# kfkq/DQMC

Measured on AMD Instinct MI355X. Metric: MC sweeps/sec, 2D Hubbard N=256 Ltau=200, higher is better.
Workload: dtype f64; 1 GPU; cfg3: 16x16 Hubbard U=8.0 beta=8.0 Ltau=200 n_stab=10 t=1 mu=-0.1; chains_per_gpu=1, n_chains_total=1, parallelism=independent chains, 1 gpu x 1 chain

## Files before the change

### dqmc_amd/abi.py

```python
from __future__ import annotations

import ctypes as C
import os
from typing import Optional, Tuple

import numpy as np

c_double_p = C.POINTER(C.c_double)
c_int64_p = C.POINTER(C.c_int64)
c_int32_p = C.POINTER(C.c_int32)
c_uint8_p = C.POINTER(C.c_uint8)
c_uint32_p = C.POINTER(C.c_uint32)
c_uint64_p = C.POINTER(C.c_uint64)


class Stats(C.Structure):
    _fields_ = [("acc_rate", C.c_double), ("max_err", C.c_double), ("sum_err", C.c_double),
                ("n_err", C.c_double), ("n_accepted", C.c_int64), ("n_proposed", C.c_int64)]

    @property
    def mean_err(self) -> float:
        return self.sum_err / self.n_err if self.n_err else 0.0


class DqmcError(RuntimeError):
    def __init__(self, code: int, msg: str):
        super().__init__(f"[{code}] {msg}")
        self.code = code


ABI_SYMBOLS = [
    "last_error", "backend", "device_count",
    "to_ldr", "ldr_mul_mat", "mat_mul_ldr", "ldr_mul_ldr", "inv_I_plus_ldr", "inv_I_plus_ldr_mul_ldr",
    "gemm", "rank1_update",
    "create", "create_batch", "n_chains", "destroy", "set_fields", "get_fields", "init", "get_G", "set_G", "get_logdet",
    "n_stack", "get_stack", "sweep_0_to_beta", "sweep_beta_to_0", "sync", "get_stats",
    "wrap_forward", "wrap_backward", "local_update_slice", "calculate_Bbar", "global_action", "set_checkerboard",
    "update_kernel_time", "set_profiling", "slice_path", "debug_snapshot", "bbar_rider_launches", "debug_gt_check",
    "measure_equal_time", "measure_accumulate", "measure_fetch",
    "sweep_unequal_time", "get_G_tau", "half_warp", "measure_unequal_time", "measure_unequal_fetch",
    "comm_unique_id", "comm_create_rccl", "comm_create_callbacks", "comm_destroy", "comm_rank", "comm_world_size",
    "comm_transport", "comm_barrier", "comm_allreduce_sum", "comm_selftest", "partner_rank", "replica_exchange_round",
    "replica_exchange_batch",
    "rng_seed", "rng_state", "rng_draw", "rng_fill_time",
]

UNIQUE_ID_BYTES = 128
SENDRECV_FN = C.CFUNCTYPE(C.c_int, C.c_void_p, C.c_void_p, C.c_void_p, C.c_size_t, C.c_int, C.c_int)


class ExchangeResult(C.Structure):
    _fields_ = [("partner", C.c_int), ("decider", C.c_int), ("accepted", C.c_int), ("pad", C.c_int),
                ("S", C.c_double), ("S_prime", C.c_double), ("S_partner", C.c_double), ("S_prime_partner", C.c_double),
# ... 69 lines not shown
            g("comm_create_callbacks").argtypes = [C.POINTER(C.c_void_p), C.c_int, C.c_int, SENDRECV_FN, C.c_void_p]
            g("comm_destroy").argtypes = [C.c_void_p]; g("comm_destroy").restype = None
            g("comm_rank").argtypes = [C.c_void_p]; g("comm_world_size").argtypes = [C.c_void_p]
            g("comm_transport").argtypes = [C.c_void_p]; g("comm_transport").restype = C.c_char_p
            g("comm_barrier").argtypes = [C.c_void_p]; g("comm_selftest").argtypes = [C.c_void_p]
            g("comm_allreduce_sum").argtypes = [C.c_void_p, c_double_p, C.c_int]
            g("partner_rank").argtypes = [C.c_int, C.c_int, C.c_int]
            g("replica_exchange_round").argtypes = [C.c_void_p, C.c_void_p, C.c_int, C.c_double, C.POINTER(ExchangeResult)]
        if self.has_symbol("replica_exchange_batch"):
            g("replica_exchange_batch").argtypes = [C.c_void_p, C.c_void_p, C.c_int, c_double_p, C.POINTER(ExchangeResult)]
        if self.has_symbol("rng_seed"):
            g("rng_seed").argtypes = [C.c_void_p, C.c_uint64, C.c_uint32, C.c_uint32]
            g("rng_state").argtypes = [C.c_void_p, c_uint64_p, c_uint32_p, c_uint32_p, C.POINTER(C.c_int)]
            g("rng_draw").argtypes = [C.c_void_p, C.c_uint32, c_int32_p, c_uint8_p, c_double_p]
            g("rng_fill_time").argtypes = [C.c_void_p, C.c_int, c_double_p]
        g("to_ldr").argtypes = [C.c_int] + [c_double_p] * 4
        g("ldr_mul_mat").argtypes = [C.c_int] + [c_double_p] * 7
        g("mat_mul_ldr").argtypes = [C.c_int] + [c_double_p] * 7
        g("ldr_mul_ldr").argtypes = [C.c_int] + [c_double_p] * 9
        g("inv_I_plus_ldr").argtypes = [C.c_int] + [c_double_p] * 5
        g("inv_I_plus_ldr_mul_ldr").argtypes = [C.c_int] + [c_double_p] * 7
        g("gemm").argtypes = [C.c_int, c_double_p, C.c_int, c_double_p, C.c_int, c_double_p]
        g("rank1_update").argtypes = [C.c_int, c_double_p, C.c_int, C.c_double]

    def _sym(self, name: str):
        return getattr(self._dll, self.prefix + name)

    def has_symbol(self, name: str) -> bool:
        return hasattr(self._dll, self.prefix + name)

# ... 41 lines not shown
        L1, d1, R1 = (_f64(x) for x in F1); L2, d2, R2 = (_f64(x) for x in F2); n = L1.shape[0]
        G = np.empty((n, n), order="F")
        self.check(self._sym("inv_I_plus_ldr_mul_ldr")(n, _p(L1), _p(d1), _p(R1), _p(L2), _p(d2), _p(R2), _p(G)))
        return G

    def gemm(self, A, B, transA: bool = False, transB: bool = False) -> np.ndarray:
        A = _f64(A); B = _f64(B); n = A.shape[0]
        Cm = np.empty((n, n), order="F")
        self.check(self._sym("gemm")(n, _p(A), int(transA), _p(B), int(transB), _p(Cm)))
        return Cm

    def rank1_update(self, G, i: int, delta: float) -> np.ndarray:
        G = np.array(G, dtype=np.float64, order="F", copy=True); n = G.shape[0]
        self.check(self._sym("rank1_update")(n, _p(G), int(i), float(delta)))
        return G

    def engine(self, *args, **kw) -> "Engine":
        return Engine(self, *args, **kw)

    def partner_rank(self, rank: int, world: int, attempt: int) -> int:
        return int(self._sym("partner_rank")(rank, world, attempt))

    def exchange_batch(self, engine: "Engine", attempt: int, u, comm: Optional["Comm"] = None) -> list:
        uv = np.ascontiguousarray(np.asarray(u, dtype=np.float64).reshape(-1))
        if uv.shape != (engine.C,):
            raise ValueError(f"u must have shape ({engine.C},), got {uv.shape}")
        res = (ExchangeResult * engine.C)()
        self.check(self._sym("replica_exchange_batch")(engine._h, comm._h if comm is not None else None, int(attempt), _p(uv), res))
        return list(res)

# ... 292 lines not shown
```

### dqmc_amd/csrc/common.h

```cpp
#pragma once

#include <hip/hip_runtime.h>
#include <cstdint>
#include <memory>
#include <string>

struct dqmc_engine;

namespace dq {

constexpr int WAVE = 64;

void set_error(const std::string& msg);
const char* get_error();

#define DQ_HIP(call)                                                                    \
    do {                                                                                \
        hipError_t _e = (call);                                                         \
        if (_e != hipSuccess) {                                                         \
            ::dq::set_error(std::string(#call) + ": " + hipGetErrorString(_e));         \
            return -2;                                              \
        }                                                                               \
    } while (0)

// ... 36 lines not shown

struct GemmDesc {
    CMat A, B;
    Mat C;
    Mat CT{nullptr, 0};
    CVec rs, ks, cs;
    int n = 0;
    int transA = 0;
    int accumulate = 0;
};
int launch_gemm(const GemmDesc& g, int n_chains, hipStream_t s);

int launch_build_expv(const int8_t* fields, long f_stride, int nt, int n, const double* tab_expv ,
                      double* expv, double* invexpv, long v_stride, int n_chains, hipStream_t s);
int launch_split_d(CVec d, Vec dl_inv, Vec ds, double* logsum, int n, int n_chains, hipStream_t s);
int launch_split_d2(CVec d1, Vec dl1, Vec ds1, CVec d2, Vec dl2, Vec ds2, int n, int n_chains, hipStream_t s);
int launch_measure_equal_time(CMat G, double* out, long out_stride, int L1, int L2, int accumulate, int n_chains, hipStream_t s);
int launch_measure_unequal_time(const double* Gtt, const double* Gt0, const double* G0t, double* out, long out_stride, int L1, int L2, int nt,
                                int accumulate, int n_chains, hipStream_t s);
int launch_axpb_identity(CMat in, Mat out, double a, double b, int n, int n_chains, hipStream_t s);
int launch_copy(CMat in, Mat out, long count, int n_chains, hipStream_t s);
int launch_set_identity(Mat out, int n, int n_chains, hipStream_t s);
int launch_transpose_scale(CMat in, Mat out, CVec rs, int n, int n_chains, hipStream_t s);
int launch_max_abs_diff(CMat A, CMat B, double* err, long err_stride, int n, int n_chains, hipStream_t s);
int launch_add_scaled_cols(CMat A, CMat B, CVec cs, Mat C, int n, int n_chains, hipStream_t s);
int launch_scale_rows(CMat in, CVec rs, Mat out, int n, int n_chains, hipStream_t s);
struct DevStats { double acc_rate, max_err, sum_err, n_err; long long n_accepted, n_proposed; };
int launch_fold_stats(DevStats* st, const int* acc, long acc_stride, int n_slices, const double* err, long err_stride, int n_err,
                      int n, int nt, int n_chains, hipStream_t s);

struct QrWork {
    double* tau; long tau_stride;
    int* jpvt; long jpvt_stride;
    unsigned long long* sync = nullptr; long sync_stride = 0;
    int* abort_words = nullptr;
    int* info = nullptr;
    double* pw = nullptr; long pw_stride = 0;
    bool pw_two_launch = false;
    int* pivpos = nullptr; long pivpos_stride = 0;
// ... 100 lines not shown
```

### dqmc_amd/csrc/elementwise.hip

```cpp
#include "common.h"
#include "wave.h"

namespace dq {

__global__ void build_expv_kernel(const int8_t* fields, long f_stride, long total, const double* tab,
                                  double* expv, double* invexpv, long v_stride) {
    const int c = blockIdx.y;
    const double* t = tab + (long)c * 8;
    for (long k = blockIdx.x * (long)blockDim.x + threadIdx.x; k < total; k += (long)gridDim.x * blockDim.x) {
        const int f = fields[(long)c * f_stride + k] & 3;
        expv[(long)c * v_stride + k] = t[f];
        invexpv[(long)c * v_stride + k] = t[4 + f];
    }
}
int launch_build_expv(const int8_t* fields, long f_stride, int nt, int n, const double* tab, double* expv, double* invexpv,
                      long v_stride, int n_chains, hipStream_t s) {
    const long total = (long)nt * n;
    dim3 grid((unsigned)((total + 255) / 256 > 512 ? 512 : (total + 255) / 256), n_chains);
    hipLaunchKernelGGL(build_expv_kernel, grid, dim3(256), 0, s, fields, f_stride, total, tab, expv, invexpv, v_stride);
    DQ_HIP(hipGetLastError());
    return 0;
}

__global__ void split_d_kernel(CVec d, Vec dl_inv, Vec ds, double* logsum, int n) {
// ... 3 lines not shown
    for (int i = threadIdx.x; i < n; i += blockDim.x) {
        const double v = dd[i];
        const bool large = v >= 1.0;
        dl_inv.at(c)[i] = large ? 1.0 / v : 1.0;
        ds.at(c)[i] = large ? 1.0 : v;
        if (large) ls += log(v);
    }
    if (logsum) {
        __shared__ double red[256];
        red[threadIdx.x] = ls;
        __syncthreads();
        for (int o = 128; o > 0; o >>= 1) { if ((int)threadIdx.x < o) red[threadIdx.x] += red[threadIdx.x + o]; __syncthreads(); }
        if (threadIdx.x == 0) logsum[c] = red[0];
    }
}
__global__ void split_d2_kernel(CVec d1, Vec dl1, Vec ds1, CVec d2, Vec dl2, Vec ds2, int n) {
    const int c = blockIdx.y;
    const double* dd = blockIdx.x ? d2.at(c) : d1.at(c);
    double* dl = blockIdx.x ? dl2.at(c) : dl1.at(c);
    double* ds = blockIdx.x ? ds2.at(c) : ds1.at(c);
    for (int i = threadIdx.x; i < n; i += blockDim.x) {
        const double v = dd[i];
        const bool large = v >= 1.0;
        dl[i] = large ? 1.0 / v : 1.0;
        ds[i] = large ? 1.0 : v;
    }
}
int launch_split_d2(CVec d1, Vec dl1, Vec ds1, CVec d2, Vec dl2, Vec ds2, int n, int n_chains, hipStream_t s) {
    hipLaunchKernelGGL(split_d2_kernel, dim3(2, n_chains), dim3(256), 0, s, d1, dl1, ds1, d2, dl2, ds2, n);
    DQ_HIP(hipGetLastError());
    return 0;
}
int launch_split_d(CVec d, Vec dl_inv, Vec ds, double* logsum, int n, int n_chains, hipStream_t s) {
    hipLaunchKernelGGL(split_d_kernel, dim3(1, n_chains), dim3(256), 0, s, d, dl_inv, ds, logsum, n);
    DQ_HIP(hipGetLastError());
    return 0;
}

__global__ void copy_kernel(CMat in, Mat out, long count) {
    const int c = blockIdx.y;
    const double* a = in.at(c); double* b = out.at(c);
    for (long k = blockIdx.x * (long)blockDim.x + threadIdx.x; k < count; k += (long)gridDim.x * blockDim.x) b[k] = a[k];
}
int launch_copy(CMat in, Mat out, long count, int n_chains, hipStream_t s) {
    long blocks = (count + 255) / 256; if (blocks > 1024) blocks = 1024;
    hipLaunchKernelGGL(copy_kernel, dim3((unsigned)blocks, n_chains), dim3(256), 0, s, in, out, count);
    DQ_HIP(hipGetLastError());
// ... 21 lines not shown
    const int tx = threadIdx.x & 31, ty = threadIdx.x >> 5;
    for (int r = ty; r < 32; r += 8) {
        const int i = ti * 32 + tx, j = tj * 32 + r;
        tile[r][tx] = (i < n && j < n) ? a[i + (long)n * j] : 0.0;
    }
    __syncthreads();
    for (int r = ty; r < 32; r += 8) {
        const int i = tj * 32 + tx, j = ti * 32 + r;
        if (i < n && j < n) {
            double v = tile[tx][r];
            if (rs.p) v *= rs.at(c)[i];
            o[i + (long)n * j] = v;
        }
    }
}
int launch_transpose_scale(CMat in, Mat out, CVec rs, int n, int n_chains, hipStream_t s) {
    const int tiles = (n + 31) / 32;
    hipLaunchKernelGGL(transpose_scale_kernel, dim3(tiles * tiles, n_chains), dim3(256), 0, s, in, out, rs, n, tiles);
    DQ_HIP(hipGetLastError());
    return 0;
}

__global__ __launch_bounds__(256) void max_abs_diff_kernel(CMat A, CMat B, double* err, long err_stride, int n) {
    const int c = blockIdx.y;
    const double* __restrict__ a = A.at(c); const double* __restrict__ b = B.at(c);
    const long total = (long)n * n;
    unsigned long long m = 0ULL;
    for (long k = (long)blockIdx.x * blockDim.x + threadIdx.x; k < total; k += (long)gridDim.x * blockDim.x) {
        const unsigned long long d = (unsigned long long)__double_as_longlong(fabs(a[k] - b[k]));
        m = d > m ? d : m;
// ... 1 lines not shown
    m = wave_max_u64(m);
    __shared__ unsigned long long red[4];
    if ((threadIdx.x & 63) == 0) red[threadIdx.x >> 6] = m;
    __syncthreads();
    if (threadIdx.x == 0) {
        unsigned long long r = red[0];
        for (int q = 1; q < 4; ++q) r = red[q] > r ? red[q] : r;
        atomicMax(reinterpret_cast<unsigned long long*>(err + (long)c * err_stride), r);
    }
}
int launch_max_abs_diff(CMat A, CMat B, double* err, long err_stride, int n, int n_chains, hipStream_t s) {
    const long total = (long)n * n;
    const long want = (total + 4095) / 4096;
    const int blocks = (int)(want < 1 ? 1 : (want > 16 ? 16 : want));
    hipLaunchKernelGGL(max_abs_diff_kernel, dim3(blocks, n_chains), dim3(256), 0, s, A, B, err, err_stride, n);
    DQ_HIP(hipGetLastError());
    return 0;
}

__global__ void add_scaled_cols_kernel(CMat A, CMat B, CVec cs, Mat C, int n) {
    const int c = blockIdx.y;
    const double* a = A.at(c); const double* b = B.at(c); double* o = C.at(c);
    const long total = (long)n * n;
    for (long k = blockIdx.x * (long)blockDim.x + threadIdx.x; k < total; k += (long)gridDim.x * blockDim.x) {
        double bv = b[k];
        if (cs.p) bv *= cs.at(c)[k / n];
        o[k] = a[k] + bv;
    }
}
int launch_add_scaled_cols(CMat A, CMat B, CVec cs, Mat C, int n, int n_chains, hipStream_t s) {
// ... 158 lines not shown
```

### dqmc_amd/csrc/engine.hip

```cpp
#include "common.h"
#include "../../include/dqmc_hip.h"

#include <cmath>
#include <cstdlib>
#include <cstring>
#include <map>
#include <memory>
#include <mutex>
#include <vector>

namespace dq {

static thread_local std::string g_err;
void set_error(const std::string& msg) { g_err = msg; }
const char* get_error() { return g_err.c_str(); }

int init_device_kernels(int device) {
    static std::mutex mu; static bool done[64] = {};
    std::lock_guard<std::mutex> lk(mu);
    if (device < 0 || device >= 64) { set_error("device ordinal out of range"); return -1; }
    if (done[device]) return 0;
    DQ_HIP(hipSetDevice(device));
    DQ_TRY(update_init_device()); DQ_TRY(update_sm_init_device()); DQ_TRY(qr_init_device()); DQ_TRY(qr_colown_init_device());
    done[device] = true;
// ... 189 lines not shown
        }
        DQ_TRY(launch_lu_blocked(M, lperm(), n, rowpos(), n, logdet_acc, 1, info(), n, C, stream));
        DQ_TRY(launch_lu_solve(M, lperm(), n, RHS, CVec(), 0, n, C, stream));
        *Y = RHS; return 0;
    }
    int inv_I_plus_ldr(LdrRef F, Mat G, double* logdet ) {
        DQ_TRY(launch_split_d(F.d, V(0), V(1), logdet, n, C, stream));
        Mat X; DQ_TRY(r_inverse_scaled(F, V(0), T(1), T(0), &X));
        DQ_TRY(launch_add_scaled_cols(X, F.L, V(1), T(2), n, C, stream));
        DQ_TRY(launch_transpose_scale(T(2), T(3), CVec(), n, C, stream));
        DQ_TRY(launch_transpose_scale(X, T(4), CVec(), n, C, stream));
        Mat Y; DQ_TRY(solve(T(3), T(4), T(0), logdet, &Y));
        return launch_transpose_scale(Y, G, CVec(), n, C, stream);
    }
    int inv_I_plus_ldr_mul_ldr(LdrRef F1, LdrRef F2, Mat G, Mat GT = Mat{nullptr, 0}) {
        DQ_TRY(launch_split_d2(F1.d, V(0), V(1), F2.d, V(2), V(3), n, C, stream));
        Mat X; DQ_TRY(r_inverse_scaled(F2, V(2), T(1), T(0), &X));
        DQ_TRY(gemm(F1.L, X, T(2), V(0), CVec(), CVec(), 1));
        DQ_TRY(gemm(F1.R, F2.L, T(2), V(1), CVec(), V(3), 0, 1));
        DQ_TRY(launch_transpose_scale(F1.L, T(3), V(0), n, C, stream));
        Mat Y; DQ_TRY(solve(T(2), T(3), T(0), nullptr, &Y));
        return gemm(X, Y, G, CVec(), CVec(), CVec(), 0, 0, GT);
    }
    int inv_invldr_plus_ldr(LdrRef F1, LdrRef F2, Mat G, bool negate) {
        DQ_TRY(launch_split_d(F1.d, V(0), V(1), nullptr, n, C, stream));
        DQ_TRY(launch_split_d(F2.d, V(2), V(3), nullptr, n, C, stream));
        Mat X; DQ_TRY(r_inverse_scaled(F2, V(2), T(1), T(0), &X));
        DQ_TRY(gemm(F1.L, X, T(2), V(0), CVec(), CVec(), 1));
        DQ_TRY(gemm(F1.R, F2.L, T(2), V(1), CVec(), V(3), 0, 1));
        DQ_TRY(launch_scale_rows(F1.R, V(1), T(3), n, C, stream));
        Mat Y; DQ_TRY(solve(T(2), T(3), T(0), nullptr, &Y));
        DQ_TRY(gemm(X, Y, G));
        if (negate) DQ_TRY(launch_axpb_identity(G, G, -1.0, 0.0, n, C, stream));
        return 0;
    }
// ... 936 lines not shown
}
int dqmc_bbar_rider_launches(dqmc_engine* h, int64_t* n_launches) {
    ENGINE_CALL(h);
    if (n_launches) *n_launches = e.rider_launches;
    return 0;
}
int dqmc_debug_gt_check(dqmc_engine* h, int on, double* max_err, int64_t* n_checks) {
    ENGINE_CALL(h); DQ_TRY(e.sync_and_check());
    if (!e.gt_err) { DQ_TRY(dev_alloc(e.gt_err, e.C)); DQ_HIP(hipMemset(e.gt_err.get(), 0, sizeof(double) * e.C)); }
    if (max_err) DQ_HIP(hipMemcpy(max_err, e.gt_err.get(), sizeof(double) * e.C, hipMemcpyDeviceToHost));
    if (n_checks) *n_checks = e.gt_checks;
    DQ_HIP(hipMemset(e.gt_err.get(), 0, sizeof(double) * e.C));
    e.gt_checks = 0; e.gt_check = on != 0;
    return 0;
}
int dqmc_slice_path(dqmc_engine* h) {
    if (!h) return -1;
    Engine& e = h->e;
    if (!is_persistent(e.slice_path)) return 0;
    unsigned solo = 0;
    for (int c = 0; c < e.C && !solo; ++c) {
        SliceSync hs; if (hipMemcpy(&hs, e.slice_sync.get() + (size_t)c * SLICE_SYNC_BYTES, 64, hipMemcpyDeviceToHost) != hipSuccess) break;
        solo = hs.solo_count;
    }
    return solo ? 2 : 1;
}
int dqmc_set_profiling(dqmc_engine* h, int on) {
    ENGINE_CALL(h); DQ_TRY(e.sync_and_check());
    e.profiling = on != 0; return 0;
}
// ... 3 lines not shown
```

### dqmc_amd/csrc/lu_gj.hip

```cpp
#include "common.h"
#include "wave.h"
#include <cstdlib>
#include <utility>

namespace dq {

namespace {
constexpr int GJ_NB = 32;
using d4 = __attribute__((ext_vector_type(4))) double;

__device__ __forceinline__ void lds_wait() { asm volatile("s_waitcnt lgkmcnt(0)" ::: "memory"); }

template <int NR, int J>
__device__ __forceinline__ void gj_step(double (&a)[NR][GJ_NB], bool (&live)[NR], int (&mypos)[NR], int& myperm, bool& singular, int lane, int k0) {
    unsigned long long best = 0ULL; int bq = -1;
#pragma unroll
    for (int q = 0; q < NR; ++q) {
        const unsigned long long kq = live[q] ? ((unsigned long long)__double_as_longlong(fabs(a[q][J])) | 1ULL) : 0ULL;
        if (kq > best) { best = kq; bq = q; }
    }
    const unsigned hi = (unsigned)(best >> 32), lo = (unsigned)best;
    const unsigned m1 = wave_max_u32(hi);
    const unsigned m2 = wave_max_u32(hi == m1 ? lo : 0u);
    const unsigned long long winners = __ballot(hi == m1 && lo == m2 && bq >= 0);
    const int pl = winners ? (int)__builtin_ctzll(winners) : 0;
    const int pq = __builtin_amdgcn_readlane(bq, pl);
    if (lane == J) myperm = pl + 64 * pq;
    double prow[GJ_NB - J];
#pragma unroll
    for (int q = 0; q < NR; ++q) {
        if (q == pq) {
#pragma unroll
            for (int c = J; c < GJ_NB; ++c) prow[c - J] = readlane_f64(a[q][c], pl);
        }
    }
#pragma unroll
    for (int q = 0; q < NR; ++q)
        if (q == pq && lane == pl) { live[q] = false; mypos[q] = k0 + J; }
    const double piv = prow[0];
// ... 96 lines not shown
        double* out = tinv + GJ_NB * GJ_NB + 256 * blk + 16 * c;
#pragma unroll
        for (int j = 0; j < 16; ++j) out[up ? 15 - j : j] = x[j];
    }
}

__device__ __forceinline__ void gj_panel_logdet(double (&LU)[GJ_NB][GJ_NB], double* logabsdet, int accumulate, int* info, int chain, int lane, int nbw, int k0, int s_sing) {
    const double pv = lane < nbw ? fabs(LU[lane][lane]) : 1.0;
    const double ls = wave_sum(log(pv));
    if (lane == 0) {
        if (logabsdet) logabsdet[chain] = ((accumulate || k0 > 0) ? logabsdet[chain] : 0.0) + ls;
        if (info && (s_sing || !(ls == ls))) atomicOr(info, DQ_STATUS_PIVOT);
    }
}
template <int... Js>
__device__ __forceinline__ void gj_tri_steps(double (&x)[16], const double* T0, int sg, int cc, bool up, bool hi, double rd, std::integer_sequence<int, Js...>) {
    auto step = [&](auto jc) {
        constexpr int j = decltype(jc)::value;
        double s0 = (j == cc) ? 1.0 : 0.0, s1 = 0.0;
#pragma unroll
        for (int m = 0; m < j; ++m) {
            const double tt = T0[sg * (j * 32 + m)];
            if (m & 1) s1 = fma(-tt, x[m], s1); else s0 = fma(-tt, x[m], s0);
        }
        const double s = s0 + s1;
        const double r0 = readlane_f64(rd, 15 - j), r1 = readlane_f64(rd, 31 - j);
        x[j] = up ? s * (hi ? r1 : r0) : s;
    };
    (step(std::integral_constant<int, Js>{}), ...);
}
__device__ __forceinline__ void gj_panel_tri_inverses(double (&LU)[GJ_NB][GJ_NB], double* inv, int lane) {
    const int blk = lane >> 4, c = lane & 15;
    const bool up = blk >= 2;
    const int base = (blk & 1) * 16;
    const double* T0 = &LU[0][0] + (up ? (base + 15) * 33 : base * 33);
    const int sg = up ? -1 : 1;
    const int cc = up ? 15 - c : c;
    const double rd = 1.0 / LU[lane & 31][lane & 31];
    double x[16];
    gj_tri_steps(x, T0, sg, cc, up, (blk & 1) != 0, rd, std::make_integer_sequence<int, 16>{});
    double* out = inv + 256 * blk + 16 * c;
#pragma unroll
    for (int j = 0; j < 16; ++j) out[up ? 15 - j : j] = x[j];
}

#ifdef DQ_GJ_STAMPS
#define GST(i) { unsigned long long t_; asm volatile("s_waitcnt lgkmcnt(0)\n\ts_memtime %0\n\ts_waitcnt lgkmcnt(0)" : "=s"(t_) :: "memory"); gst[i] += t_ - gprev; gprev = t_; }
#define GST_ARGS , unsigned long long (&gst)[8], unsigned long long& gprev
#define GST_PASS , gst, gprev
#else
#define GST(i)
#define GST_ARGS
#define GST_PASS
#endif
template <int J, int NW, int RPL>
// ... 3 lines not shown
    constexpr int C0 = J & ~1;
    GST(0)
    double aj = a[0][J]; int bs = 0;
    if (RPL > 1) asm volatile("" : "+v"(aj));
    unsigned long long key = (live & 1u) ? ((unsigned long long)__double_as_longlong(fabs(aj)) | 1ULL) : 0ULL;
#pragma unroll
    for (int q = 1; q < RPL; ++q) {
        double v = a[q][J];
        asm volatile("" : "+v"(v));
        const unsigned long long kq = ((live >> q) & 1u) ? ((unsigned long long)__double_as_longlong(fabs(v)) | 1ULL) : 0ULL;
        if (kq > key) { key = kq; aj = v; bs = q; }
    }
    double rme = __builtin_amdgcn_rcp(aj);
    rme = fma(fma(-aj, rme, 1.0), rme, rme);
    rme = fma(fma(-aj, rme, 1.0), rme, rme);
    const unsigned hi = (unsigned)(key >> 32), lo = (unsigned)key;
    const unsigned m1 = wave_max_u32(hi);
    const unsigned m2 = wave_max_u32(hi == m1 ? lo : 0u);
    const unsigned long long winners = __ballot(hi == m1 && lo == m2 && key != 0ULL);
    const int cl = winners ? (int)__builtin_ctzll(winners) : 0;
    GST(1)
    if (lane == cl) {
#pragma unroll
        for (int q = 0; q < RPL; ++q) {
            if (bs == q) {
#pragma unroll
                for (int c = C0; c < GJ_NB; c += 2) *reinterpret_cast<double2*>(&slot_row[PAR][wave][c]) = make_double2(a[q][c], a[q][c + 1]);
            }
        }
        slot_row[PAR][wave][GJ_NB] = rme;
        slot_key[PAR][wave] = winners ? ((((unsigned long long)m1 << 32) | m2) & ~0x1FFULL) | (unsigned long long)(cl | (bs << 6)) | 0x100ULL : 0ULL;
    }
    GST(2)
    asm volatile("s_waitcnt lgkmcnt(0)" ::: "memory");
    __builtin_amdgcn_s_barrier();
    asm volatile("" ::: "memory");
    GST(3)
    constexpr int NWK = (NW + 1) & ~1;
    ulonglong2 kp[NWK / 2];
#pragma unroll
    for (int q = 0; q < NWK / 2; ++q) kp[q] = *reinterpret_cast<const ulonglong2*>(&slot_key[PAR][2 * q]);
    unsigned long long best = kp[0].x; int pw = 0;
    if ((kp[0].y >> 9) > (best >> 9)) { best = kp[0].y; pw = 1; }
#pragma unroll
    for (int q = 1; q < NWK / 2; ++q) {
        if ((kp[q].x >> 9) > (best >> 9)) { best = kp[q].x; pw = 2 * q; }
// ... 451 lines not shown
        else if (n > 512) DQ_GJ_PANEL(3, 3);
        else if (n > 256) DQ_GJ_PANEL(4, 2);
        else if (n > 64) DQ_GJ_PANEL(4, 1);
        else hipLaunchKernelGGL((gj_panel_kernel<1>), pg, dim3(64), 0, s, CMat(A), rowpos, rowpos_stride, perm, perm_stride, tinv, logabsdet, accumulate_logdet, info, n, k0);
        const int nbw = n - k0 < GJ_NB ? n - k0 : GJ_NB;
        const int nA = (n + 31) / 32, nS = k0 / 32;
        const int nCA = (n - k0 - nbw + 31) / 32, nCB = (n + 31) / 32;
        hipLaunchKernelGGL(gj_update_kernel, dim3((nA + nS + 1) * (nCA + nCB), n_chains), dim3(256), 0, s, A, B, SA, X, (const int*)rowpos, rowpos_stride,
                           (const int*)perm, perm_stride, (const double*)tinv, n, k0, nA, nS, nCA);
    }
#undef DQ_GJ_PANEL
    DQ_HIP(hipGetLastError());
    return 0;
}

}
```

### dqmc_amd/csrc/qr_panel.hip

```cpp
#include "common.h"
#include "wave.h"
#include <utility>

namespace dq {

namespace {

#ifdef DQ_QP_STAMPS
#define QST(i) { unsigned long long t_; asm volatile("s_memtime %0\n\ts_waitcnt lgkmcnt(0)" : "=s"(t_) :: "memory"); if (threadIdx.x == 0) qst[i] = t_; }
#else
#define QST(i)
#endif

constexpr int QP_B = 16;
constexpr int QP_SR = 32;
#ifndef QP_SEL_ROWS
#define QP_SEL_ROWS 32
#endif
constexpr int QP_SEL = QP_SEL_ROWS;
typedef double d4 __attribute__((ext_vector_type(4)));

__device__ __forceinline__ unsigned qp_row_bits(unsigned r) {
    unsigned h = r * 0x9E3779B1u + 0x85EBCA77u;
    h ^= h >> 16; h *= 0x85EBCA6Bu; h ^= h >> 13; h *= 0xC2B2AE35u; h ^= h >> 16;
// ... 10 lines not shown
    const double e = __hiloint2double((int)h16[0], (int)l16[0]), o = __hiloint2double((int)h16[1], (int)l16[1]);
    const double s = e + o;
    const unsigned slo = (unsigned)__double_as_longlong(s), shi = (unsigned)(__double_as_longlong(s) >> 32);
    auto l32 = __builtin_amdgcn_permlane32_swap(slo, slo, false, false);
    auto h32 = __builtin_amdgcn_permlane32_swap(shi, shi, false, false);
    return __hiloint2double((int)h32[0], (int)l32[0]) + __hiloint2double((int)h32[1], (int)l32[1]);
}

template <int J>
__device__ __forceinline__ void dpp_fmac_self(double& d, double a) {
    asm volatile("v_fmac_f64_dpp %0, %1, %1 row_newbcast:%2 row_mask:0xf bank_mask:0xf" : "+v"(d) : "v"(a), "n"(J));
}
template <int J>
__device__ __forceinline__ void dpp_axpy_self(double& a, double m) {
    asm volatile("v_fmac_f64_dpp %0, %0, %1 row_newbcast:%2 row_mask:0xf bank_mask:0xf" : "+v"(a) : "v"(m), "n"(J));
}
__device__ __forceinline__ void dpp_fence(double (&a)[16]) {
    asm volatile("s_nop 1" : "+v"(a[0]), "+v"(a[1]), "+v"(a[2]), "+v"(a[3]), "+v"(a[4]), "+v"(a[5]), "+v"(a[6]), "+v"(a[7]),
                             "+v"(a[8]), "+v"(a[9]), "+v"(a[10]), "+v"(a[11]), "+v"(a[12]), "+v"(a[13]), "+v"(a[14]), "+v"(a[15]));
}

__device__ __forceinline__ void dpp_fence1(double& z) { asm volatile("s_nop 1" : "+v"(z)); }
template <int T>
__device__ __forceinline__ void dpp_fmac(double& d, double z, double y) {
    asm volatile("v_fmac_f64_dpp %0, %1, %2 row_newbcast:%3 row_mask:0xf bank_mask:0xf" : "+v"(d) : "v"(z), "v"(y), "n"(T));
}
template <int... Ts>
__device__ __forceinline__ void t_row_dot(double& tj, const double (&trow)[16], double z, std::integer_sequence<int, Ts...>) {
    (dpp_fmac<Ts>(tj, z, trow[Ts]), ...);
}

template <int NW>
struct PanelShared {
    static constexpr int NWP = NW < 2 ? 2 : NW;
    alignas(16) unsigned long long key[2][NWP];
    alignas(16) double cand[2][QP_SEL + 2];
    alignas(16) double part[2][QP_B][NWP];
    alignas(16) double prow[2][QP_B];
    int sel[QP_B];
};
// ... 724 lines not shown
```

### dqmc_amd/csrc/wave.h

```cpp
#pragma once
#include <hip/hip_runtime.h>

namespace dq {

template <int CTRL, int ROW_MASK>
__device__ __forceinline__ double dpp_mov_f64(double x) {
    const long long b = __double_as_longlong(x);
    const int lo = __builtin_amdgcn_update_dpp(0, (int)(b & 0xffffffffLL), CTRL, ROW_MASK, 0xf, false);
    const int hi = __builtin_amdgcn_update_dpp(0, (int)(b >> 32), CTRL, ROW_MASK, 0xf, false);
    return __longlong_as_double(((long long)hi << 32) | (unsigned int)lo);
}

__device__ __forceinline__ double readlane_f64(double x, int lane ) {
    const long long b = __double_as_longlong(x);
    const int lo = __builtin_amdgcn_readlane((int)(b & 0xffffffffLL), lane);
    const int hi = __builtin_amdgcn_readlane((int)(b >> 32), lane);
    return __longlong_as_double(((long long)hi << 32) | (unsigned int)lo);
}

__device__ __forceinline__ double wave_sum(double x) {
    x += dpp_mov_f64<0xB1, 0xf>(x);
    x += dpp_mov_f64<0x4E, 0xf>(x);
    x += dpp_mov_f64<0x141, 0xf>(x);
    x += dpp_mov_f64<0x140, 0xf>(x);
// ... 23 lines not shown
    DQ_MAX32(0x141, 0xf)
    DQ_MAX32(0x140, 0xf)
    DQ_MAX32(0x142, 0xa)
    DQ_MAX32(0x143, 0xc)
#undef DQ_MAX32
    return (unsigned)__builtin_amdgcn_readlane((int)k, 63);
}

__device__ __forceinline__ unsigned long long wave_max_u64(unsigned long long k) {
    const unsigned hi = (unsigned)(k >> 32), lo = (unsigned)k;
    const unsigned m1 = wave_max_u32(hi);
    const unsigned m2 = wave_max_u32(hi == m1 ? lo : 0u);
    return ((unsigned long long)m1 << 32) | m2;
}

}
```

### include/dqmc_hip.h

```cpp
#ifndef DQMC_HIP_H
#define DQMC_HIP_H

#include <stddef.h>
#include <stdint.h>

#ifdef __cplusplus
extern "C" {
#endif

#define DQMC_OK         0
#define DQMC_EINVAL    -1
#define DQMC_ENODEVICE -2
#define DQMC_ENUMERIC  -3
#define DQMC_ERANGE    -4
#define DQMC_ENOMEM    -5

typedef struct dqmc_engine dqmc_engine;

typedef struct dqmc_stats {
    double  acc_rate;
    double  max_err;
    double  sum_err;
    double  n_err;
    int64_t n_accepted;
// ... 114 lines not shown
    double S_prime_partner;
    double deltaS;
} dqmc_exchange_result;

int dqmc_replica_exchange_round(dqmc_engine* e, dqmc_comm* comm, int exchange_attempt, double u,
                                dqmc_exchange_result* result);

int dqmc_replica_exchange_batch(dqmc_engine* e, dqmc_comm* comm, int exchange_attempt, const double* u,
                                dqmc_exchange_result* result);

int dqmc_update_kernel_time(dqmc_engine* e, double* ms, int64_t* n_launches, int64_t* n_accepted);
int dqmc_slice_path(dqmc_engine* e);
int dqmc_debug_snapshot(dqmc_engine* e, double* wrap_err, int* accepted, unsigned int* sync_words, unsigned int* slice_epoch);
int dqmc_bbar_rider_launches(dqmc_engine* e, int64_t* n_launches);
int dqmc_debug_gt_check(dqmc_engine* e, int on, double* max_err, int64_t* n_checks);
int dqmc_set_profiling(dqmc_engine* e, int on);

#ifdef __cplusplus
}
#endif
#endif
```

Measured before the change: 13.37 sweeps/s.

## Fuse split_d2 with scaled transpose; fast wave argmax; DPP triangular inverse in GJ

Merges the diagonal-split kernel with the scaled transpose of L1 into one launch, so inv_I_plus_ldr_mul_ldr issues one fewer kernel. It adds a wave-wide u64 max-with-winners helper that skips the second reduction when the top 32 bits already pick a single lane, and uses it in the LU/GJ pivot searches. It also rewrites the panel triangular inverse to preload the negated row values into registers and accumulate with DPP broadcast FMAs instead of repeated LDS reads. Debug entry points are added to check the new routines against reference forms; the DPP path depends on inline-asm hazard fences being placed correctly.

```diff
diff --git a/dqmc_amd/abi.py b/dqmc_amd/abi.py
--- a/dqmc_amd/abi.py
+++ b/dqmc_amd/abi.py
@@ -37,6 +37,7 @@
     "n_stack", "get_stack", "sweep_0_to_beta", "sweep_beta_to_0", "sync", "get_stats",
     "wrap_forward", "wrap_backward", "local_update_slice", "calculate_Bbar", "global_action", "set_checkerboard",
     "update_kernel_time", "set_profiling", "slice_path", "debug_snapshot", "bbar_rider_launches", "debug_gt_check",
+    "debug_wave_max_u64", "debug_gj_tri_inverses",
     "measure_equal_time", "measure_accumulate", "measure_fetch",
     "sweep_unequal_time", "get_G_tau", "half_warp", "measure_unequal_time", "measure_unequal_fetch",
     "comm_unique_id", "comm_create_rccl", "comm_create_callbacks", "comm_destroy", "comm_rank", "comm_world_size",
@@ -136,6 +137,9 @@
             g("rng_state").argtypes = [C.c_void_p, c_uint64_p, c_uint32_p, c_uint32_p, C.POINTER(C.c_int)]
             g("rng_draw").argtypes = [C.c_void_p, C.c_uint32, c_int32_p, c_uint8_p, c_double_p]
             g("rng_fill_time").argtypes = [C.c_void_p, C.c_int, c_double_p]
+        if self.has_symbol("debug_wave_max_u64"):
+            g("debug_wave_max_u64").argtypes = [c_uint64_p, C.c_int, C.c_int, c_uint64_p]
+            g("debug_gj_tri_inverses").argtypes = [c_double_p, C.c_int, C.c_int, c_double_p]
         g("to_ldr").argtypes = [C.c_int] + [c_double_p] * 4
         g("ldr_mul_mat").argtypes = [C.c_int] + [c_double_p] * 7
         g("mat_mul_ldr").argtypes = [C.c_int] + [c_double_p] * 7
@@ -207,6 +211,22 @@
         G = np.array(G, dtype=np.float64, order="F", copy=True); n = G.shape[0]
         self.check(self._sym("rank1_update")(n, _p(G), int(i), float(delta)))
         return G
+
+    def debug_wave_max_u64(self, keys, form: int) -> Tuple[np.ndarray, np.ndarray]:
+        keys = np.ascontiguousarray(keys, dtype=np.uint64)
+        if keys.ndim != 2 or keys.shape[1] != 64:
+            raise ValueError(f"keys must have shape (k, 64), got {keys.shape}")
+        out = np.zeros((keys.shape[0], 2), dtype=np.uint64)
+        self.check(self._sym("debug_wave_max_u64")(keys.ctypes.data_as(c_uint64_p), keys.shape[0], int(form), out.ctypes.data_as(c_uint64_p)))
+        return out[:, 0].copy(), out[:, 1].copy()
+
+    def debug_gj_tri_inverses(self, LU, form: int) -> np.ndarray:
+        LU = np.ascontiguousarray(LU, dtype=np.float64)
+        if LU.ndim != 3 or LU.shape[1:] != (32, 32):
+            raise ValueError(f"LU must have shape (k, 32, 32), got {LU.shape}")
+        inv = np.zeros((LU.shape[0], 4, 16, 16))
+        self.check(self._sym("debug_gj_tri_inverses")(_p(LU), LU.shape[0], int(form), _p(inv)))
+        return np.ascontiguousarray(inv.transpose(0, 1, 3, 2))
 
     def engine(self, *args, **kw) -> "Engine":
         return Engine(self, *args, **kw)
diff --git a/dqmc_amd/csrc/common.h b/dqmc_amd/csrc/common.h
--- a/dqmc_amd/csrc/common.h
+++ b/dqmc_amd/csrc/common.h
@@ -74,7 +74,7 @@
 int launch_build_expv(const int8_t* fields, long f_stride, int nt, int n, const double* tab_expv ,
                       double* expv, double* invexpv, long v_stride, int n_chains, hipStream_t s);
 int launch_split_d(CVec d, Vec dl_inv, Vec ds, double* logsum, int n, int n_chains, hipStream_t s);
-int launch_split_d2(CVec d1, Vec dl1, Vec ds1, CVec d2, Vec dl2, Vec ds2, int n, int n_chains, hipStream_t s);
+int launch_split_d2_rhs(CVec d1, Vec dl1, Vec ds1, CVec d2, Vec dl2, Vec ds2, CMat L1, Mat rhs, int n, int n_chains, hipStream_t s);
 int launch_measure_equal_time(CMat G, double* out, long out_stride, int L1, int L2, int accumulate, int n_chains, hipStream_t s);
 int launch_measure_unequal_time(const double* Gtt, const double* Gt0, const double* G0t, double* out, long out_stride, int L1, int L2, int nt,
                                 int accumulate, int n_chains, hipStream_t s);
@@ -83,6 +83,8 @@
 int launch_set_identity(Mat out, int n, int n_chains, hipStream_t s);
 int launch_transpose_scale(CMat in, Mat out, CVec rs, int n, int n_chains, hipStream_t s);
 int launch_max_abs_diff(CMat A, CMat B, double* err, long err_stride, int n, int n_chains, hipStream_t s);
+int launch_debug_wave_max(const unsigned long long* keys, int k, int form, unsigned long long* out, hipStream_t s);
+int launch_gj_debug_tri_inverses(const double* LU, int k, int form, double* inv, hipStream_t s);
 int launch_add_scaled_cols(CMat A, CMat B, CVec cs, Mat C, int n, int n_chains, hipStream_t s);
 int launch_scale_rows(CMat in, CVec rs, Mat out, int n, int n_chains, hipStream_t s);
 struct DevStats { double acc_rate, max_err, sum_err, n_err; long long n_accepted, n_proposed; };
diff --git a/dqmc_amd/csrc/elementwise.hip b/dqmc_amd/csrc/elementwise.hip
--- a/dqmc_amd/csrc/elementwise.hip
+++ b/dqmc_amd/csrc/elementwise.hip
@@ -41,23 +41,6 @@
         if (threadIdx.x == 0) logsum[c] = red[0];
     }
 }
-__global__ void split_d2_kernel(CVec d1, Vec dl1, Vec ds1, CVec d2, Vec dl2, Vec ds2, int n) {
-    const int c = blockIdx.y;
-    const double* dd = blockIdx.x ? d2.at(c) : d1.at(c);
-    double* dl = blockIdx.x ? dl2.at(c) : dl1.at(c);
-    double* ds = blockIdx.x ? ds2.at(c) : ds1.at(c);
-    for (int i = threadIdx.x; i < n; i += blockDim.x) {
-        const double v = dd[i];
-        const bool large = v >= 1.0;
-        dl[i] = large ? 1.0 / v : 1.0;
-        ds[i] = large ? 1.0 : v;
-    }
-}
-int launch_split_d2(CVec d1, Vec dl1, Vec ds1, CVec d2, Vec dl2, Vec ds2, int n, int n_chains, hipStream_t s) {
-    hipLaunchKernelGGL(split_d2_kernel, dim3(2, n_chains), dim3(256), 0, s, d1, dl1, ds1, d2, dl2, ds2, n);
-    DQ_HIP(hipGetLastError());
-    return 0;
-}
 int launch_split_d(CVec d, Vec dl_inv, Vec ds, double* logsum, int n, int n_chains, hipStream_t s) {
     hipLaunchKernelGGL(split_d_kernel, dim3(1, n_chains), dim3(256), 0, s, d, dl_inv, ds, logsum, n);
     DQ_HIP(hipGetLastError());
@@ -109,6 +92,44 @@
         }
     }
 }
+__global__ void split_d2_rhs_kernel(CVec d1, Vec dl1, Vec ds1, CVec d2, Vec dl2, Vec ds2, CMat L1, Mat rhs, int n, int tiles) {
+    __shared__ double tile[32][33];
+    const int c = blockIdx.y;
+    const int b = blockIdx.x - tiles * tiles;
+    if (b >= 0) {
+        const double* dd = b ? d2.at(c) : d1.at(c);
+        double* dl = b ? dl2.at(c) : dl1.at(c);
+        double* ds = b ? ds2.at(c) : ds1.at(c);
+        for (int i = threadIdx.x; i < n; i += blockDim.x) {
+            const double v = dd[i];
+            const bool large = v >= 1.0;
+            dl[i] = large ? 1.0 / v : 1.0;
+            ds[i] = large ? 1.0 : v;
+        }
+        return;
+    }
+    const double* a = L1.at(c); double* o = rhs.at(c);
+    const int ti = blockIdx.x % tiles, tj = blockIdx.x / tiles;
+    const int tx = threadIdx.x & 31, ty = threadIdx.x >> 5;
+    for (int r = ty; r < 32; r += 8) {
+        const int i = ti * 32 + tx, j = tj * 32 + r;
+        tile[r][tx] = (i < n && j < n) ? a[i + (long)n * j] : 0.0;
+    }
+    const int io = tj * 32 + tx;
+    const double v1 = d1.at(c)[io < n ? io : 0];
+    const double sc = v1 >= 1.0 ? 1.0 / v1 : 1.0;
+    __syncthreads();
+    for (int r = ty; r < 32; r += 8) {
+        const int j = ti * 32 + r;
+        if (io < n && j < n) o[io + (long)n * j] = tile[tx][r] * sc;
+    }
+}
+int launch_split_d2_rhs(CVec d1, Vec dl1, Vec ds1, CVec d2, Vec dl2, Vec ds2, CMat L1, Mat rhs, int n, int n_chains, hipStream_t s) {
+    const int tiles = (n + 31) / 32;
+    hipLaunchKernelGGL(split_d2_rhs_kernel, dim3(tiles * tiles + 2, n_chains), dim3(256), 0, s, d1, dl1, ds1, d2, dl2, ds2, L1, rhs, n, tiles);
+    DQ_HIP(hipGetLastError());
+    return 0;
+}
 int launch_transpose_scale(CMat in, Mat out, CVec rs, int n, int n_chains, hipStream_t s) {
     const int tiles = (n + 31) / 32;
     hipLaunchKernelGGL(transpose_scale_kernel, dim3(tiles * tiles, n_chains), dim3(256), 0, s, in, out, rs, n, tiles);
@@ -140,6 +161,23 @@
     const long want = (total + 4095) / 4096;
     const int blocks = (int)(want < 1 ? 1 : (want > 16 ? 16 : want));
     hipLaunchKernelGGL(max_abs_diff_kernel, dim3(blocks, n_chains), dim3(256), 0, s, A, B, err, err_stride, n);
+    DQ_HIP(hipGetLastError());
+    return 0;
+}
+
+__global__ __launch_bounds__(64) void debug_wave_max_kernel(const unsigned long long* __restrict__ keys, int form, unsigned long long* out) {
+    const unsigned long long k = keys[(long)blockIdx.x * 64 + threadIdx.x];
+    unsigned long long m, w;
+    if (form == 1) m = wave_max_u64_winners(k, w);
+    else {
+        m = wave_max_u64(k);
+        w = __ballot(k == m && k != 0ULL);
+    }
+    if (threadIdx.x == 0) { out[2L * blockIdx.x] = m; out[2L * blockIdx.x + 1] = w; }
+}
+int launch_debug_wave_max(const unsigned long long* keys, int k, int form, unsigned long long* out, hipStream_t s) {
+    if (k <= 0) return 0;
+    hipLaunchKernelGGL(debug_wave_max_kernel, dim3(k), dim3(64), 0, s, keys, form, out);
     DQ_HIP(hipGetLastError());
     return 0;
 }
diff --git a/dqmc_amd/csrc/engine.hip b/dqmc_amd/csrc/engine.hip
--- a/dqmc_amd/csrc/engine.hip
+++ b/dqmc_amd/csrc/engine.hip
@@ -227,11 +227,10 @@
         return launch_transpose_scale(Y, G, CVec(), n, C, stream);
     }
     int inv_I_plus_ldr_mul_ldr(LdrRef F1, LdrRef F2, Mat G, Mat GT = Mat{nullptr, 0}) {
-        DQ_TRY(launch_split_d2(F1.d, V(0), V(1), F2.d, V(2), V(3), n, C, stream));
+        DQ_TRY(launch_split_d2_rhs(F1.d, V(0), V(1), F2.d, V(2), V(3), F1.L, T(3), n, C, stream));
         Mat X; DQ_TRY(r_inverse_scaled(F2, V(2), T(1), T(0), &X));
         DQ_TRY(gemm(F1.L, X, T(2), V(0), CVec(), CVec(), 1));
         DQ_TRY(gemm(F1.R, F2.L, T(2), V(1), CVec(), V(3), 0, 1));
-        DQ_TRY(launch_transpose_scale(F1.L, T(3), V(0), n, C, stream));
         Mat Y; DQ_TRY(solve(T(2), T(3), T(0), nullptr, &Y));
         return gemm(X, Y, G, CVec(), CVec(), CVec(), 0, 0, GT);
     }
@@ -1198,6 +1197,32 @@
     e.gt_checks = 0; e.gt_check = on != 0;
     return 0;
 }
+static int debug_device() {
+    int count = 0;
+    if (hipGetDeviceCount(&count) != hipSuccess || count == 0) { set_error("no HIP device available: this library requires a gfx950 GPU"); return DQMC_ENODEVICE; }
+    DQ_HIP(hipSetDevice(0));
+    return 0;
+}
+int dqmc_debug_wave_max_u64(const uint64_t* keys, int k, int form, uint64_t* out) {
+    if (!keys || !out || k < 1 || form < 0 || form > 1) { set_error("debug_wave_max_u64: keys, out, k >= 1 and form 0 or 1"); return DQMC_EINVAL; }
+    DQ_TRY(debug_device());
+    DevPtr<unsigned long long> dk, dout;
+    DQ_TRY(dev_alloc(dk, (size_t)64 * k)); DQ_TRY(dev_alloc(dout, (size_t)2 * k));
+    DQ_HIP(hipMemcpy(dk.get(), keys, sizeof(uint64_t) * 64 * k, hipMemcpyHostToDevice));
+    DQ_TRY(launch_debug_wave_max(dk.get(), k, form, dout.get(), nullptr));
+    DQ_HIP(hipMemcpy(out, dout.get(), sizeof(uint64_t) * 2 * k, hipMemcpyDeviceToHost));
+    return 0;
+}
+int dqmc_debug_gj_tri_inverses(const double* LU, int k, int form, double* inv) {
+    if (!LU || !inv || k < 1 || form < 0 || form > 1) { set_error("debug_gj_tri_inverses: LU, inv, k >= 1 and form 0 or 1"); return DQMC_EINVAL; }
+    DQ_TRY(debug_device());
+    DevPtr<double> dlu, dinv;
+    DQ_TRY(dev_alloc(dlu, (size_t)1024 * k)); DQ_TRY(dev_alloc(dinv, (size_t)1024 * k));
+    DQ_HIP(hipMemcpy(dlu.get(), LU, sizeof(double) * 1024 * k, hipMemcpyHostToDevice));
+    DQ_TRY(launch_gj_debug_tri_inverses(dlu.get(), k, form, dinv.get(), nullptr));
+    DQ_HIP(hipMemcpy(inv, dinv.get(), sizeof(double) * 1024 * k, hipMemcpyDeviceToHost));
+    return 0;
+}
 int dqmc_slice_path(dqmc_engine* h) {
     if (!h) return -1;
     Engine& e = h->e;
diff --git a/dqmc_amd/csrc/lu_gj.hip b/dqmc_amd/csrc/lu_gj.hip
--- a/dqmc_amd/csrc/lu_gj.hip
+++ b/dqmc_amd/csrc/lu_gj.hip
@@ -19,10 +19,8 @@
         const unsigned long long kq = live[q] ? ((unsigned long long)__double_as_longlong(fabs(a[q][J])) | 1ULL) : 0ULL;
         if (kq > best) { best = kq; bq = q; }
     }
-    const unsigned hi = (unsigned)(best >> 32), lo = (unsigned)best;
-    const unsigned m1 = wave_max_u32(hi);
-    const unsigned m2 = wave_max_u32(hi == m1 ? lo : 0u);
-    const unsigned long long winners = __ballot(hi == m1 && lo == m2 && bq >= 0);
+    unsigned long long winners;
+    wave_max_u64_winners(best, winners);
     const int pl = winners ? (int)__builtin_ctzll(winners) : 0;
     const int pq = __builtin_amdgcn_readlane(bq, pl);
     if (lane == J) myperm = pl + 64 * pq;
@@ -149,7 +147,7 @@
     }
 }
 template <int... Js>
-__device__ __forceinline__ void gj_tri_steps(double (&x)[16], const double* T0, int sg, int cc, bool up, bool hi, double rd, std::integer_sequence<int, Js...>) {
+__device__ __forceinline__ void gj_tri_steps_ref(double (&x)[16], const double* T0, int sg, int cc, bool up, bool hi, double rd, std::integer_sequence<int, Js...>) {
     auto step = [&](auto jc) {
         constexpr int j = decltype(jc)::value;
         double s0 = (j == cc) ? 1.0 : 0.0, s1 = 0.0;
@@ -164,7 +162,7 @@
     };
     (step(std::integral_constant<int, Js>{}), ...);
 }
-__device__ __forceinline__ void gj_panel_tri_inverses(double (&LU)[GJ_NB][GJ_NB], double* inv, int lane) {
+__device__ __forceinline__ void gj_panel_tri_inverses_ref(double (&LU)[GJ_NB][GJ_NB], double* inv, int lane) {
     const int blk = lane >> 4, c = lane & 15;
     const bool up = blk >= 2;
     const int base = (blk & 1) * 16;
@@ -173,7 +171,41 @@
     const int cc = up ? 15 - c : c;
     const double rd = 1.0 / LU[lane & 31][lane & 31];
     double x[16];
-    gj_tri_steps(x, T0, sg, cc, up, (blk & 1) != 0, rd, std::make_integer_sequence<int, 16>{});
+    gj_tri_steps_ref(x, T0, sg, cc, up, (blk & 1) != 0, rd, std::make_integer_sequence<int, 16>{});
+    double* out = inv + 256 * blk + 16 * c;
+#pragma unroll
+    for (int j = 0; j < 16; ++j) out[up ? 15 - j : j] = x[j];
+}
+template <int... Ms>
+__device__ __forceinline__ void gj_tri_dot(double& s0, double& s1, double nt, const double (&x)[16], std::integer_sequence<int, Ms...>) {
+    (dpp_fmac<Ms>((Ms & 1) ? s1 : s0, nt, x[Ms]), ...);
+}
+template <int... Js>
+__device__ __forceinline__ void gj_tri_steps(double (&x)[16], double (&nt)[16], int cc, bool up, bool hi, double rd, std::integer_sequence<int, Js...>) {
+    auto step = [&](auto jc) {
+        constexpr int j = decltype(jc)::value;
+        double s0 = (j == cc) ? 1.0 : 0.0, s1 = 0.0;
+        gj_tri_dot(s0, s1, nt[j], x, std::make_integer_sequence<int, j>{});
+        const double s = s0 + s1;
+        const double r0 = readlane_f64(rd, 15 - j), r1 = readlane_f64(rd, 31 - j);
+        x[j] = up ? s * (hi ? r1 : r0) : s;
+    };
+    (step(std::integral_constant<int, Js>{}), ...);
+}
+__device__ __forceinline__ void gj_panel_tri_inverses(double (&LU)[GJ_NB][GJ_NB], double* inv, int lane) {
+    const int blk = lane >> 4, c = lane & 15;
+    const bool up = blk >= 2;
+    const int base = (blk & 1) * 16;
+    const double* T0 = &LU[0][0] + (up ? (base + 15) * 33 : base * 33);
+    const int sg = up ? -1 : 1;
+    const int cc = up ? 15 - c : c;
+    double nt[16];
+#pragma unroll
+    for (int j = 0; j < 16; ++j) nt[j] = -T0[sg * (j * 32 + c)];
+    const double rd = 1.0 / LU[lane & 31][lane & 31];
+    dpp_fence(nt);
+    double x[16];
+    gj_tri_steps(x, nt, cc, up, (blk & 1) != 0, rd, std::make_integer_sequence<int, 16>{});
     double* out = inv + 256 * blk + 16 * c;
 #pragma unroll
     for (int j = 0; j < 16; ++j) out[up ? 15 - j : j] = x[j];
@@ -207,10 +239,8 @@
     double rme = __builtin_amdgcn_rcp(aj);
     rme = fma(fma(-aj, rme, 1.0), rme, rme);
     rme = fma(fma(-aj, rme, 1.0), rme, rme);
-    const unsigned hi = (unsigned)(key >> 32), lo = (unsigned)key;
-    const unsigned m1 = wave_max_u32(hi);
-    const unsigned m2 = wave_max_u32(hi == m1 ? lo : 0u);
-    const unsigned long long winners = __ballot(hi == m1 && lo == m2 && key != 0ULL);
+    unsigned long long winners;
+    const unsigned long long wmax = wave_max_u64_winners(key, winners);
     const int cl = winners ? (int)__builtin_ctzll(winners) : 0;
     GST(1)
     if (lane == cl) {
@@ -222,7 +252,7 @@
             }
         }
         slot_row[PAR][wave][GJ_NB] = rme;
-        slot_key[PAR][wave] = winners ? ((((unsigned long long)m1 << 32) | m2) & ~0x1FFULL) | (unsigned long long)(cl | (bs << 6)) | 0x100ULL : 0ULL;
+        slot_key[PAR][wave] = winners ? (wmax & ~0x1FFULL) | (unsigned long long)(cl | (bs << 6)) | 0x100ULL : 0ULL;
     }
     GST(2)
     asm volatile("s_waitcnt lgkmcnt(0)" ::: "memory");
@@ -704,4 +734,24 @@
     return 0;
 }
 
-}
+namespace {
+template <int FORM>
+__global__ __launch_bounds__(64) void gj_debug_tri_kernel(const double* __restrict__ LUs, double* invs) {
+    __shared__ __attribute__((aligned(16))) double LU[GJ_NB][GJ_NB];
+    const int lane = threadIdx.x;
+    const double* src = LUs + (long)blockIdx.x * GJ_NB * GJ_NB;
+    for (int e = lane; e < GJ_NB * GJ_NB; e += 64) (&LU[0][0])[e] = src[e];
+    __syncthreads();
+    double* inv = invs + (long)blockIdx.x * GJ_NB * GJ_NB;
+    if (FORM == 0) gj_panel_tri_inverses_ref(LU, inv, lane); else gj_panel_tri_inverses(LU, inv, lane);
+}
+}
+int launch_gj_debug_tri_inverses(const double* LU, int k, int form, double* inv, hipStream_t s) {
+    if (k <= 0) return 0;
+    if (form == 0) hipLaunchKernelGGL(gj_debug_tri_kernel<0>, dim3(k), dim3(64), 0, s, LU, inv);
+    else hipLaunchKernelGGL(gj_debug_tri_kernel<1>, dim3(k), dim3(64), 0, s, LU, inv);
+    DQ_HIP(hipGetLastError());
+    return 0;
+}
+
+}
diff --git a/dqmc_amd/csrc/qr_panel.hip b/dqmc_amd/csrc/qr_panel.hip
--- a/dqmc_amd/csrc/qr_panel.hip
+++ b/dqmc_amd/csrc/qr_panel.hip
@@ -48,16 +48,6 @@
 template <int J>
 __device__ __forceinline__ void dpp_axpy_self(double& a, double m) {
     asm volatile("v_fmac_f64_dpp %0, %0, %1 row_newbcast:%2 row_mask:0xf bank_mask:0xf" : "+v"(a) : "v"(m), "n"(J));
-}
-__device__ __forceinline__ void dpp_fence(double (&a)[16]) {
-    asm volatile("s_nop 1" : "+v"(a[0]), "+v"(a[1]), "+v"(a[2]), "+v"(a[3]), "+v"(a[4]), "+v"(a[5]), "+v"(a[6]), "+v"(a[7]),
-                             "+v"(a[8]), "+v"(a[9]), "+v"(a[10]), "+v"(a[11]), "+v"(a[12]), "+v"(a[13]), "+v"(a[14]), "+v"(a[15]));
-}
-
-__device__ __forceinline__ void dpp_fence1(double& z) { asm volatile("s_nop 1" : "+v"(z)); }
-template <int T>
-__device__ __forceinline__ void dpp_fmac(double& d, double z, double y) {
-    asm volatile("v_fmac_f64_dpp %0, %1, %2 row_newbcast:%3 row_mask:0xf bank_mask:0xf" : "+v"(d) : "v"(z), "v"(y), "n"(T));
 }
 template <int... Ts>
 __device__ __forceinline__ void t_row_dot(double& tj, const double (&trow)[16], double z, std::integer_sequence<int, Ts...>) {
diff --git a/dqmc_amd/csrc/wave.h b/dqmc_amd/csrc/wave.h
--- a/dqmc_amd/csrc/wave.h
+++ b/dqmc_amd/csrc/wave.h
@@ -61,4 +61,30 @@
     return ((unsigned long long)m1 << 32) | m2;
 }
 
+__device__ __forceinline__ unsigned long long wave_max_u64_winners(unsigned long long k, unsigned long long& winners) {
+    const unsigned hi = (unsigned)(k >> 32), lo = (unsigned)k;
+    const unsigned long long nonzero = __builtin_amdgcn_ballot_w64(k != 0ULL);
+    const unsigned m1 = wave_max_u32(hi);
+    const unsigned long long top = __builtin_amdgcn_ballot_w64(hi == m1) & nonzero;
+    unsigned m2;
+    if (__builtin_expect((top & (top - 1ULL)) != 0ULL, 0)) {
+        m2 = wave_max_u32(hi == m1 ? lo : 0u);
+        winners = __builtin_amdgcn_ballot_w64(lo == m2) & top;
+    } else {
+        m2 = (unsigned)__builtin_amdgcn_readlane((int)lo, top ? (int)__builtin_ctzll(top) : 0);
+        winners = top;
+    }
+    return ((unsigned long long)m1 << 32) | m2;
 }
+
+__device__ __forceinline__ void dpp_fence1(double& z) { asm volatile("s_nop 1" : "+v"(z)); }
+__device__ __forceinline__ void dpp_fence(double (&a)[16]) {
+    asm volatile("s_nop 1" : "+v"(a[0]), "+v"(a[1]), "+v"(a[2]), "+v"(a[3]), "+v"(a[4]), "+v"(a[5]), "+v"(a[6]), "+v"(a[7]),
+                             "+v"(a[8]), "+v"(a[9]), "+v"(a[10]), "+v"(a[11]), "+v"(a[12]), "+v"(a[13]), "+v"(a[14]), "+v"(a[15]));
+}
+template <int T>
+__device__ __forceinline__ void dpp_fmac(double& d, double z, double y) {
+    asm volatile("v_fmac_f64_dpp %0, %1, %2 row_newbcast:%3 row_mask:0xf bank_mask:0xf" : "+v"(d) : "v"(z), "v"(y), "n"(T));
+}
+
+}
diff --git a/include/dqmc_hip.h b/include/dqmc_hip.h
--- a/include/dqmc_hip.h
+++ b/include/dqmc_hip.h
@@ -152,6 +152,8 @@
 int dqmc_debug_snapshot(dqmc_engine* e, double* wrap_err, int* accepted, unsigned int* sync_words, unsigned int* slice_epoch);
 int dqmc_bbar_rider_launches(dqmc_engine* e, int64_t* n_launches);
 int dqmc_debug_gt_check(dqmc_engine* e, int on, double* max_err, int64_t* n_checks);
+int dqmc_debug_wave_max_u64(const uint64_t* keys, int k, int form, uint64_t* out);
+int dqmc_debug_gj_tri_inverses(const double* LU, int k, int form, double* inv);
 int dqmc_set_profiling(dqmc_engine* e, int on);
 
 #ifdef __cplusplus
```

After: 13.44 sweeps/s (median of 6 runs). About the same (+0.5%).
